# kurtosis/mat_mul

Hardware: NVIDIA B200
Metric: env_steps_per_sec (higher is better)
Workload: dtype int8

## Files before the change

### mat_mul_b200/csrc/tg_common.cuh

```cuda
#pragma once
#include <cuda_runtime.h>
#include <stdint.h>

#include <type_traits>

#include "../../include/tensorgame.h"

namespace tg {

template <int S>
struct Geo {
    static constexpr int S2 = S * S;
    static constexpr int S3 = S2 * S;
    static constexpr int RP = (S2 + 3) & ~3;
    static constexpr int WR = RP / 4;
    static constexpr int GP = (S * RP + 15) & ~15;
    static constexpr int TP = (3 * S + 15) & ~15;
    static constexpr bool STRADDLE = (S % 4) != 0;
};

__host__ __device__ constexpr bool supported_S(int S) { return S == 4 || S == 9 || S == 16 || S == 25; }
__host__ __device__ constexpr bool basis_supported_S(int S) { return S == 4 || S == 9 || S == 16; }

extern int g_last_cuda_error;

#ifdef TG_TUNING
}
#include <cstdlib>
namespace tg {
inline int tuning_env(const char *name, int dflt) {
    const char *e = getenv(name);
    return e ? atoi(e) : dflt;
}
#endif

inline int cuda_fail(cudaError_t e) {
    g_last_cuda_error = (int)e;
    return TG_E_CUDA;
}
#define TG_CUDA(call)                                  \
    do {                                               \
        cudaError_t _e = (call);                       \
        if (_e != cudaSuccess) return tg::cuda_fail(_e); \
    } while (0)

int sm_count();

template <class F>
int with_S(int S, F &&f) {
    switch (S) {
    case 4: return f(std::integral_constant<int, 4>{});
    case 9: return f(std::integral_constant<int, 9>{});
    case 16: return f(std::integral_constant<int, 16>{});
    case 25: return f(std::integral_constant<int, 25>{});
    }
    return TG_E_ARG;
}

constexpr int LAUNCH = 1;

inline bool misaligned(const void *p, uintptr_t align) { return ((uintptr_t)p & (align - 1)) != 0; }

inline int check_step(int S, long long B, int shift, const void *in, const void *tape, const void *out, const void *flags,
                      const void *nnz) {
    if (!supported_S(S) || B < 0 || shift < 1 || shift > 4) return TG_E_ARG;
    if (B == 0) return TG_OK;
    if (!in || !tape || !out || !flags || !nnz) return TG_E_ARG;
    if (misaligned(in, 16) || misaligned(out, 16) || misaligned(tape, 16)) return TG_E_ARG;
    return LAUNCH;
}

inline int check_expand(int S, long long B, int k, int shift, const void *parents, const void *tape, const void *children,
                        const void *flags, const void *nnz) {
    if (k < 1) return TG_E_ARG;
    return check_step(S, B, shift, parents, tape, children, flags, nnz);
}

inline int check_rollout(int S, long long B, int K, int shift, const void *in, const void *tape, long long stride, const void *out,
                         const void *flags, const void *nnz, const void *steps, bool freeze) {
    if (!supported_S(S) || B < 0 || K < 0 || shift < 1 || shift > 4) return TG_E_ARG;
    if (B == 0) return TG_OK;
    if (!in || !out || !flags || !nnz || (freeze && !steps) || (K > 0 && !tape)) return TG_E_ARG;
    if (misaligned(in, 16) || misaligned(out, 16) || misaligned(tape, 16) || (stride & 15)) return TG_E_ARG;
    return LAUNCH;
}

inline int check_pair(int S, long long B, const void *src, uintptr_t src_align, const void *dst, uintptr_t dst_align) {
    if (!supported_S(S) || B < 0) return TG_E_ARG;
    if (B == 0) return TG_OK;
    if (!src || !dst) return TG_E_ARG;
    if (misaligned(src, src_align) || misaligned(dst, dst_align)) return TG_E_ARG;
    return LAUNCH;
}

inline int check_basis_gf2(int S, long long N, const void *in, const void *mats, const void *out) {
    if (!supported_S(S) || N < 0) return TG_E_ARG;
    if (N == 0) return TG_OK;
    if (!in || !mats || !out) return TG_E_ARG;
    if (misaligned(in, 16) || misaligned(out, 16) || misaligned(mats, 4)) return TG_E_ARG;
    return LAUNCH;
}

inline int check_basis_factors_gf2(int S, long long N, int R, int shift_in, int shift_out, const void *tape_in, long long in_stride,
                                   const void *mats, const void *tape_out, long long out_stride) {
    if (!supported_S(S) || N < 0 || R < 1 || shift_in < 1 || shift_in > 4 || shift_out < 1 || shift_out > 4) return TG_E_ARG;
    if (N == 0) return TG_OK;
    if (!tape_in || !mats || !tape_out) return TG_E_ARG;
    if (misaligned(tape_in, 16) || misaligned(tape_out, 16) || (in_stride & 15) || (out_stride & 15) || misaligned(mats, 4)) return TG_E_ARG;
    return LAUNCH;
}

inline int check_sample_gf2(int S, long long N, double p_nonzero, const void *mats) {
    if (!supported_S(S) || N < 0 || !(p_nonzero >= 0.0 && p_nonzero <= 1.0)) return TG_E_ARG;
    if (N == 0) return TG_OK;
    if (!mats) return TG_E_ARG;
    if (misaligned(mats, 4)) return TG_E_ARG;
    return LAUNCH;
}

inline int check_demo_sample_gf2(int S, long long N, int R, int dim_t, int replay_shift, long long nb, const void *tape_dm,
                                 const void *targets, const void *idx, const void *states, const void *scalars, const void *actions,
                                 const void *rewards) {
    if (!supported_S(S) || N < 0 || R < 1 || dim_t < 1 || nb < 0) return TG_E_ARG;
    if (nb == 0) return TG_OK;
    if (!tape_dm || !targets || !idx || !states || !scalars || !actions || !rewards) return TG_E_ARG;
    if (misaligned(tape_dm, 16) || misaligned(targets, 16)) return TG_E_ARG;
    if (replay_shift < 0 || replay_shift > 8) return TG_E_ARG;
    return LAUNCH;
}

constexpr uint8_t BASIS_REDO = 0x80;
int launch_basis_mma16(const int8_t *slab_in, const int8_t *mats, long long mat_stride, void *slab_out, int out16, uint8_t *flags,
                       long long N, cudaStream_t st);
int launch_basis_mma9(const int8_t *slab_in, const int8_t *mats, long long mat_stride, void *slab_out, int out16, uint8_t *flags,
                      long long N, cudaStream_t st);

int launch_rollout_rows(const int8_t *slab_in, const uint8_t *tape, long long stride, int K, int8_t *slab_out, uint8_t *flags,
                        int32_t *nnz, int32_t *steps, long long B, int S, int shift, int freeze, cudaStream_t st);
bool demo_acc16_mma_applies(int R);
int launch_demo_acc16_mma(const uint8_t *tape, long long tape_step_stride, long long N, int R, int shift, int8_t *slab,
                          uint8_t *flags, int or_flags, cudaStream_t st);

__device__ __forceinline__ void philox_block(uint32_t c0, uint32_t c1, uint32_t c2, uint32_t c3, uint32_t k0, uint32_t k1,
                                             uint32_t out[4]) {
#pragma unroll
    for (int r = 0; r < 10; r++) {
        const uint32_t hi0 = __umulhi(0xD2511F53u, c0), lo0 = 0xD2511F53u * c0;
        const uint32_t hi1 = __umulhi(0xCD9E8D57u, c2), lo1 = 0xCD9E8D57u * c2;
        c0 = hi1 ^ c1 ^ k0, c1 = lo1, c2 = hi0 ^ c3 ^ k1, c3 = lo0;
        k0 += 0x9E3779B9u, k1 += 0xBB67AE85u;
    }
    out[0] = c0, out[1] = c1, out[2] = c2, out[3] = c3;
}

__device__ __forceinline__ unsigned long long splitmix64(unsigned long long z) {
    z += 0x9E3779B97F4A7C15ull;
    z = (z ^ (z >> 30)) * 0xBF58476D1CE4E5B9ull;
    z = (z ^ (z >> 27)) * 0x94D049BB133111EBull;
    return z ^ (z >> 31);
}
__device__ __forceinline__ unsigned long long key_const(unsigned base, int i) { return splitmix64((unsigned long long)(base + i)) | 1ull; }

__device__ __forceinline__ uint32_t smem_u32(const void *p) { return (uint32_t)__cvta_generic_to_shared(p); }

__device__ __forceinline__ void mbar_init(uint64_t *bar, uint32_t count) {
    asm volatile("mbarrier.init.shared::cta.b64 [%0], %1;" ::"r"(smem_u32(bar)), "r"(count));
}
__device__ __forceinline__ void mbar_fence_init() { asm volatile("fence.mbarrier_init.release.cluster;" ::: "memory"); }
__device__ __forceinline__ void mbar_expect_tx(uint64_t *bar, uint32_t bytes) {
    asm volatile("mbarrier.arrive.expect_tx.shared::cta.b64 _, [%0], %1;" ::"r"(smem_u32(bar)), "r"(bytes) : "memory");
}
__device__ __forceinline__ void mbar_wait(uint64_t *bar, uint32_t parity) {
    asm volatile(
        "{\n"
        ".reg .pred p;\n"
        "WAIT_%=:\n"
        "mbarrier.try_wait.parity.shared::cta.b64 p, [%0], %1;\n"
        "@p bra DONE_%=;\n"
        "bra WAIT_%=;\n"
        "DONE_%=:\n"
        "}\n" ::"r"(smem_u32(bar)),
        "r"(parity)
        : "memory");
}
__device__ __forceinline__ void bulk_g2s(void *dst_smem, const void *src_gmem, uint32_t bytes, uint64_t *bar) {
    asm volatile("cp.async.bulk.shared::cluster.global.mbarrier::complete_tx::bytes [%0], [%1], %2, [%3];" ::"r"(
                     smem_u32(dst_smem)),
                 "l"(src_gmem), "r"(bytes), "r"(smem_u32(bar))
                 : "memory");
}
__device__ __forceinline__ void bulk_s2g(void *dst_gmem, const void *src_smem, uint32_t bytes) {
    asm volatile("cp.async.bulk.global.shared::cta.bulk_group [%0], [%1], %2;" ::"l"(dst_gmem), "r"(smem_u32(src_smem)),
                 "r"(bytes)
                 : "memory");
}
__device__ __forceinline__ void bulk_commit() { asm volatile("cp.async.bulk.commit_group;" ::: "memory"); }
template <int N>
__device__ __forceinline__ void bulk_wait_read() {
    asm volatile("cp.async.bulk.wait_group.read %0;" ::"n"(N) : "memory");
}
template <int N>
__device__ __forceinline__ void bulk_wait() {
    asm volatile("cp.async.bulk.wait_group %0;" ::"n"(N) : "memory");
}
__device__ __forceinline__ void fence_proxy_async() { asm volatile("fence.proxy.async.shared::cta;" ::: "memory"); }

constexpr uint32_t H4 = 0x80808080u;
constexpr uint32_t ONES4 = 0x01010101u;

__device__ __forceinline__ uint32_t nonzero_mask(uint32_t x) { return (((x & 0x7F7F7F7Fu) + 0x7F7F7F7Fu) | x) & H4; }

__device__ __forceinline__ uint32_t byte_sum(uint32_t x) { return __dp4a(x, ONES4, 0u); }

__device__ __forceinline__ void st_f32x4(float *p, float a, float b, float c, float d) {
    asm volatile("st.global.v4.f32 [%0], {%1, %2, %3, %4};" ::"l"(__cvta_generic_to_global(p)), "f"(a), "f"(b), "f"(c), "f"(d) : "memory");
}
__device__ __forceinline__ void st_f32x2(float *p, float a, float b) {
    asm volatile("st.global.v2.f32 [%0], {%1, %2};" ::"l"(__cvta_generic_to_global(p)), "f"(a), "f"(b) : "memory");
}
__device__ __forceinline__ void st_f32(float *p, float a) {
    asm volatile("st.global.f32 [%0], %1;" ::"l"(__cvta_generic_to_global(p)), "f"(a) : "memory");
}
__device__ __forceinline__ void ld_f32x4(const float *p, float f[4]) {
    asm volatile("ld.global.nc.v4.f32 {%0, %1, %2, %3}, [%4];" : "=f"(f[0]), "=f"(f[1]), "=f"(f[2]), "=f"(f[3]) : "l"(__cvta_generic_to_global(p)));
}
__device__ __forceinline__ void ld_f32x2(const float *p, float &a, float &b) {
    asm volatile("ld.global.nc.v2.f32 {%0, %1}, [%2];" : "=f"(a), "=f"(b) : "l"(__cvta_generic_to_global(p)));
}
__device__ __forceinline__ float ld_f32(const float *p) {
    float a;
    asm volatile("ld.global.nc.f32 %0, [%1];" : "=f"(a) : "l"(__cvta_generic_to_global(p)));
    return a;
}

template <int S>
__device__ __forceinline__ void store_run(float *p, int nv, float a, float b, float c, float d) {
    const uint32_t lo = (uint32_t)reinterpret_cast<uintptr_t>(p);
    if constexpr (Geo<S>::S2 % 4 == 0) {
        if ((lo & 15u) == 0) {
            st_f32x4(p, a, b, c, d);
            return;
        }
    }
    if (nv == 4) {
        if ((lo & 7u) == 0) {
            st_f32x2(p, a, b);
            st_f32x2(p + 2, c, d);
        } else {
            st_f32(p, a);
            st_f32x2(p + 1, b, c);
            st_f32(p + 3, d);
        }
    } else {
        if (nv > 0) st_f32(p, a);
        if (nv > 1) st_f32(p + 1, b);
        if (nv > 2) st_f32(p + 2, c);
    }
}

template <int S>
__device__ __forceinline__ void load_run(const float *p, int nv, float f[4]) {
    const uint32_t lo = (uint32_t)reinterpret_cast<uintptr_t>(p);
    f[0] = f[1] = f[2] = f[3] = 0.f;
    if constexpr (Geo<S>::S2 % 4 == 0) {
        if ((lo & 15u) == 0) {
            ld_f32x4(p, f);
            return;
        }
    }
    if (nv == 4) {
        if ((lo & 7u) == 0) {
            ld_f32x2(p, f[0], f[1]);
            ld_f32x2(p + 2, f[2], f[3]);
        } else {
            f[0] = ld_f32(p);
            ld_f32x2(p + 1, f[1], f[2]);
            f[3] = ld_f32(p + 3);
        }
    } else {
        if (nv > 0) f[0] = ld_f32(p);
        if (nv > 1) f[1] = ld_f32(p + 1);
        if (nv > 2) f[2] = ld_f32(p + 2);
    }
}

}
```

### mat_mul_b200/csrc/tg_expand.cu

```cuda
#include "tg_step.cuh"

namespace tg {

template <int B>
__device__ __forceinline__ int sext_byte_e(uint32_t w) {
    constexpr uint32_t sel = (uint32_t)B | ((uint32_t)(B | 8) << 4) | ((uint32_t)(B | 8) << 8) | ((uint32_t)(B | 8) << 12);
    uint32_t d;
    asm("prmt.b32 %0, %1, %2, %3;" : "=r"(d) : "r"(w), "r"(0u), "r"(sel));
    return (int)d;
}
__device__ __forceinline__ unsigned long long quad_sum64(unsigned long long x) {
    x += __shfl_xor_sync(0xFFFFFFFFu, x, 1);
    x += __shfl_xor_sync(0xFFFFFFFFu, x, 2);
    return x;
}

template <bool KEYS>
__global__ void __launch_bounds__(128)
    expand4_rows_kernel(const int8_t *__restrict__ parents, const uint8_t *__restrict__ tape, int k, int8_t *__restrict__ children,
                        uint8_t *__restrict__ flags, int32_t *__restrict__ nnz, unsigned long long *__restrict__ keys, long long B,
                        int shift) {
    constexpr int S = 4;
    const long long gt = (long long)blockIdx.x * blockDim.x + threadIdx.x;
    const long long b = min(gt >> 2, B - 1);
    const bool real = (gt >> 2) < B;
    const int i = (int)(gt & 3);
    uint32_t row[4];
    {
        const uint4 t = __ldg(reinterpret_cast<const uint4 *>(parents + b * 64) + i);
        row[0] = t.x ^ H4, row[1] = t.y ^ H4, row[2] = t.z ^ H4, row[3] = t.w ^ H4;
    }
    unsigned long long pkey = 0;
    const unsigned long long Ai = i == 0 ? key_const(0x1000, 0) : i == 1 ? key_const(0x1000, 1) : i == 2 ? key_const(0x1000, 2) : key_const(0x1000, 3);
    if constexpr (KEYS) {
        unsigned long long ti = 0;
#pragma unroll
        for (int j = 0; j < S; j++) {
            const uint32_t w = row[j] ^ H4;
            unsigned long long sij = 0;
#pragma unroll
            for (int kk = 0; kk < S; kk++) sij += (unsigned long long)(long long)(int8_t)(w >> (8 * kk)) * key_const(0x3000, kk);
            ti += sij * key_const(0x2000, j);
        }
        pkey = quad_sum64(ti * Ai);
    }
    const uint32_t sh4 = (uint32_t)shift * ONES4, tokmax = (uint32_t)(0x7F - 2 * shift) * ONES4;
    const uint4 *rec = reinterpret_cast<const uint4 *>(tape + b * k * 16);
    uint4 *dst = reinterpret_cast<uint4 *>(children + b * k * 64) + i;
    const int ush = 8 * i;
    unsigned long long kc[S] = {0, 0, 0, 0};
    if constexpr (KEYS) {
#pragma unroll
        for (int x = 0; x < S; x++) kc[x] = key_const(0x1000u * (unsigned)(i + 1), x);
    }
    uint4 q = __ldg(rec);
    for (int c = 0; c < k; c++) {
        const uint4 cur = q;
        if (c + 1 < k) q = __ldg(rec + c + 1);
        const uint32_t over = ((((cur.x & 0x7F7F7F7Fu) + tokmax) | cur.x) | (((cur.y & 0x7F7F7F7Fu) + tokmax) | cur.y) |
                               (((cur.z & 0x7F7F7F7Fu) + tokmax) | cur.z)) & H4;
        const uint32_t cu = ((cur.x | H4) - sh4) ^ H4, cv = ((cur.y | H4) - sh4) ^ H4, cw = ((cur.z | H4) - sh4) ^ H4;
        const int wi = (int)(cur.z - sh4);
        const int ui = (int)(int8_t)(cu >> ush);
        const int v[4] = {sext_byte_e<0>(cv), sext_byte_e<1>(cv), sext_byte_e<2>(cv), sext_byte_e<3>(cv)};
        uint32_t part = 0, rng = 0;
        uint32_t t[4];
#pragma unroll
        for (int j = 0; j < 4; j++) {
            const uint32_t x = (row[j] - (uint32_t)(ui * v[j] * wi)) ^ H4;
            t[j] = x;
            part += (uint32_t)__popc(nonzero_mask(x));
            rng |= x ^ (x << 1);
        }
        if (real) dst[4 * c] = make_uint4(t[0], t[1], t[2], t[3]);
        part |= (rng & H4) != 0 ? 1u << 16 : 0u;
        part += __shfl_xor_sync(0xFFFFFFFFu, part, 1);
        part += __shfl_xor_sync(0xFFFFFFFFu, part, 2);
        unsigned long long fkey = 0;
        if constexpr (KEYS) {
            const uint32_t cm = i == 0 ? cu : (i == 1 ? cv : cw);
            unsigned long long f = 0;
#pragma unroll
            for (int x = 0; x < S; x++) f += (unsigned long long)(long long)(int8_t)(cm >> (8 * x)) * kc[x];
            const unsigned long long f1 = __shfl_sync(0xFFFFFFFFu, f, (threadIdx.x & 28) | 1);
            const unsigned long long f2 = __shfl_sync(0xFFFFFFFFu, f, (threadIdx.x & 28) | 2);
            fkey = f * f1 * f2;
        }
        if (real && i == 0) {
            const uint32_t cntv = part & 0xFFFFu;
            const bool changed = cu != 0 && cv != 0 && cw != 0;
            const long long child = b * k + c;
            flags[child] = (uint8_t)((cntv == 0 ? TG_FLAG_TERMINAL : 0u) | (changed ? 0u : TG_FLAG_NULL) |
                                     (((part >> 16) != 0 || over != 0) ? TG_FLAG_RANGE : 0u));
            nnz[child] = (int32_t)cntv;
            if constexpr (KEYS) keys[child] = pkey - fkey;
        }
    }
}

}

extern "C" int tg_expand_children(const int8_t *parents, const uint8_t *tape, int k, int8_t *children, uint8_t *flags,
                                  int32_t *nnz, uint64_t *keys, int64_t B, int S, int shift, void *stream) {
    if (const int rc = tg::check_expand(S, B, k, shift, parents, tape, children, flags, nnz); rc != tg::LAUNCH) return rc;
    cudaStream_t st = (cudaStream_t)stream;
    switch (S) {
    case 4: {
#ifdef TG_TUNING
        if (tg::tuning_env("TG_EXPAND_COLUMNS", 0))
            return tg::launch_expand<4, 256, tg::W8>(parents, tape, k, children, flags, nnz, (unsigned long long *)keys, B, shift, st);
#endif
        const long long grid = (B * 4 + 127) / 128;
        if (grid > 0x7FFFFFFFLL) return TG_E_ARG;
        if (keys) tg::expand4_rows_kernel<true><<<(int)grid, 128, 0, st>>>(parents, tape, k, children, flags, nnz, (unsigned long long *)keys, B, shift);
        else tg::expand4_rows_kernel<false><<<(int)grid, 128, 0, st>>>(parents, tape, k, children, flags, nnz, nullptr, B, shift);
        TG_CUDA(cudaGetLastError());
        return TG_OK;
    }
    case 9: return tg::launch_expand<9, 128, tg::W8>(parents, tape, k, children, flags, nnz, (unsigned long long *)keys, B, shift, st);
    case 16: return tg::launch_expand<16, 128, tg::W8>(parents, tape, k, children, flags, nnz, (unsigned long long *)keys, B, shift, st);
    case 25: return tg::launch_expand<25, 160, tg::W8>(parents, tape, k, children, flags, nnz, (unsigned long long *)keys, B, shift, st);
    }
    return TG_E_ARG;
}
```

### mat_mul_b200/csrc/tg_step.cu

```cuda
#include "tg_step.cuh"

namespace tg {

int g_last_cuda_error = 0;

int sm_count() {
    static int cached[64] = {0};
    int dev = 0;
    if (cudaGetDevice(&dev) != cudaSuccess || dev < 0 || dev >= 64) return 148;
    if (!cached[dev]) {
        int n = 0;
        if (cudaDeviceGetAttribute(&n, cudaDevAttrMultiProcessorCount, dev) != cudaSuccess || n <= 0) n = 148;
        cached[dev] = n;
    }
    return cached[dev];
}

#ifdef TG_TUNING
static int g_step_ctas_per_sm = 0;
static int g_step_variant = 0;
#endif

static int step_ctas_per_sm(int n) {
#ifdef TG_TUNING
    if (g_step_ctas_per_sm > 0) return g_step_ctas_per_sm;
#endif
    return n;
}

}

extern "C" {

int tg_version(void) { return TG_VERSION; }
int tg_last_cuda_error(void) { return tg::g_last_cuda_error; }

const char *tg_error_string(int code) {
    switch (code) {
    case TG_OK: return "ok";
    case TG_E_ARG: return "bad argument";
    case TG_E_CUDA: return "CUDA runtime error (see tg_last_cuda_error)";
    case TG_E_RANGE: return "value does not fit the device format";
    default: return "unknown error";
    }
}

int tg_layout(int S, int *row_pitch, int *game_pitch, int *token_pitch) {
    if (!tg::supported_S(S)) return TG_E_ARG;
    const int rp = (S * S + 3) & ~3;
    if (row_pitch) *row_pitch = rp;
    if (game_pitch) *game_pitch = (S * rp + 15) & ~15;
    if (token_pitch) *token_pitch = (3 * S + 15) & ~15;
    return TG_OK;
}

#ifdef TG_TUNING
int tg_tune_step_ctas_per_sm(int n) {
    tg::g_step_ctas_per_sm = n;
    return TG_OK;
}
int tg_tune_step_variant(int v) {
    tg::g_step_variant = v;
    return TG_OK;
}
#endif

int tg_step(const int8_t *slab_in, const uint8_t *tape, int8_t *slab_out, uint8_t *flags, int32_t *nnz, int64_t B, int S,
            int shift, void *stream) {
    if (const int rc = tg::check_step(S, B, shift, slab_in, tape, slab_out, flags, nnz); rc != tg::LAUNCH) return rc;
    cudaStream_t st = (cudaStream_t)stream;
#ifdef TG_TUNING
    switch (S * 10 + tg::g_step_variant) {
    case 41: return tg::launch_step<4, 256, 2, 2, tg::W8>(slab_in, tape, slab_out, flags, nnz, B, shift, tg::step_ctas_per_sm(32), st);
    case 42: return tg::launch_step<4, 256, 4, 3, tg::W8>(slab_in, tape, slab_out, flags, nnz, B, shift, tg::step_ctas_per_sm(32), st);
    case 43: return tg::launch_step<4, 256, 8, 2, tg::W8>(slab_in, tape, slab_out, flags, nnz, B, shift, tg::step_ctas_per_sm(32), st);
    case 91: return tg::launch_step<9, 256, 1, 3, tg::W8>(slab_in, tape, slab_out, flags, nnz, B, shift, tg::step_ctas_per_sm(5), st);
    case 92: return tg::launch_step<9, 256, 1, 4, tg::W8>(slab_in, tape, slab_out, flags, nnz, B, shift, tg::step_ctas_per_sm(5), st);
    case 93: return tg::launch_step<9, 256, 4, 2, tg::W8>(slab_in, tape, slab_out, flags, nnz, B, shift, tg::step_ctas_per_sm(32), st);
    case 94: return tg::launch_step<9, 512, 1, 3, tg::W8>(slab_in, tape, slab_out, flags, nnz, B, shift, tg::step_ctas_per_sm(3), st);
    case 95: return tg::launch_step<9, 128, 2, 3, tg::W8>(slab_in, tape, slab_out, flags, nnz, B, shift, tg::step_ctas_per_sm(7), st);
    case 96: return tg::launch_step<9, 128, 4, 3, tg::W8>(slab_in, tape, slab_out, flags, nnz, B, shift, tg::step_ctas_per_sm(5), st);
    case 97: return tg::launch_step<9, 256, 2, 3, tg::W8>(slab_in, tape, slab_out, flags, nnz, B, shift, tg::step_ctas_per_sm(32), st);
    case 161: return tg::launch_step<16, 256, 1, 3, tg::W8>(slab_in, tape, slab_out, flags, nnz, B, shift, tg::step_ctas_per_sm(32), st);
    case 162: return tg::launch_step<16, 256, 2, 2, tg::W8>(slab_in, tape, slab_out, flags, nnz, B, shift, tg::step_ctas_per_sm(32), st);
    case 163: return tg::launch_step<16, 512, 1, 2, tg::W8>(slab_in, tape, slab_out, flags, nnz, B, shift, tg::step_ctas_per_sm(32), st);
    default: break;
    }
#endif
    switch (S) {
    case 4: return tg::launch_step<4, 256, 4, 2, tg::W8>(slab_in, tape, slab_out, flags, nnz, B, shift, tg::step_ctas_per_sm(32), st);
    case 9: return tg::launch_step<9, 256, 2, 2, tg::W8>(slab_in, tape, slab_out, flags, nnz, B, shift, tg::step_ctas_per_sm(32), st);
    case 16: return tg::launch_step<16, 256, 1, 2, tg::W8>(slab_in, tape, slab_out, flags, nnz, B, shift, tg::step_ctas_per_sm(32), st);
    case 25: return tg::launch_step<25, 160, 1, 2, tg::W8>(slab_in, tape, slab_out, flags, nnz, B, shift, tg::step_ctas_per_sm(32), st);
    }
    return TG_E_ARG;
}

}
```

### mat_mul_b200/csrc/tg_step.cuh

```cuda
#pragma once
#include "tg_common.cuh"

namespace tg {

struct W8 {
    using T = int8_t;
    static constexpr int EB = 1;
    static constexpr uint32_t H = H4;
    static constexpr int NB = 16, CB = 8;
    static constexpr bool UNROLL_PASSES = true;

    template <int S>
    struct Lane {
        int c;
        uint32_t hv;
        uint32_t maskA;
        uint32_t maskB;
        int off_vA, off_vB;
        int off_w[4];
        int tokw;

        __device__ __forceinline__ void init(int c_) {
            using G = Geo<S>;
            c = c_;
            tokw = c_ % (G::TP / 4);
            const int jk0 = 4 * c;
            const int jA = jk0 / S;
            hv = 0, maskA = 0, maskB = 0;
#pragma unroll
            for (int b = 0; b < 4; b++) {
                const int jk = jk0 + b;
                const bool valid = jk < G::S2;
                const int j = valid ? jk / S : jA;
                const int k = valid ? jk % S : 0;
                off_w[b] = 2 * S + k;
                if (valid) {
                    hv |= 0x80u << (8 * b);
                    if (j == jA)
                        maskA |= 0xFFu << (8 * b);
                    else
                        maskB |= 0xFFu << (8 * b);
                }
            }
            off_vA = S + jA;
            off_vB = S + (jA + 1 < S ? jA + 1 : jA);
        }
    };

    template <int S>
    static __device__ __forceinline__ int32_t pack_vw(const uint8_t *tok, const Lane<S> &L, int shift) {
        using G = Geo<S>;
        const int vA = (int)tok[L.off_vA] - shift;
        if constexpr (!G::STRADDLE) {
            const uint32_t wt = *reinterpret_cast<const uint32_t *>(tok + L.off_w[0]);
            return vA * (int32_t)(wt - (uint32_t)shift * ONES4);
        } else {
            const int vB = (int)tok[L.off_vB] - shift;
            const uint32_t wt = (uint32_t)tok[L.off_w[0]] | ((uint32_t)tok[L.off_w[1]] << 8) |
                                ((uint32_t)tok[L.off_w[2]] << 16) | ((uint32_t)tok[L.off_w[3]] << 24);
            const uint32_t sh = (uint32_t)shift * ONES4, mv = L.maskA | L.maskB;
            const int32_t ws = (int32_t)((wt & mv) - (sh & mv));
            const int32_t wsB = (int32_t)((wt & L.maskB) - (sh & L.maskB));
            return vA * ws + (vB - vA) * wsB;
        }
    }

    static __device__ __forceinline__ uint32_t lane_sum(uint32_t cnt) { return byte_sum(cnt); }

    template <int S>
    struct ColumnKey {
        unsigned long long kb[4];

        __device__ __forceinline__ void init(int c) {
#pragma unroll
            for (int q = 0; q < 4; q++) {
                const int jk = 4 * c + q;
                kb[q] = jk < Geo<S>::S2 ? key_const(0x2000, jk / S) * key_const(0x3000, jk % S) : 0ull;
            }
        }
        __device__ __forceinline__ unsigned long long operator()(const uint32_t (&row)[S]) const {
            unsigned long long a0 = 0;
#pragma unroll
            for (int i = 0; i < S; i++) a0 -= 128ull * key_const(0x1000, i);
            unsigned long long acc[4] = {a0, a0, a0, a0};
#pragma unroll
            for (int i = 0; i < S; i++) {
#pragma unroll
                for (int q = 0; q < 4; q++) acc[q] += (unsigned long long)((row[i] >> (8 * q)) & 0xFFu) * key_const(0x1000, i);
            }
            return acc[0] * kb[0] + acc[1] * kb[1] + acc[2] * kb[2] + acc[3] * kb[3];
        }
    };
};

struct W16 {
    using T = int16_t;
    static constexpr int EB = 2;
    static constexpr uint32_t H = 0x80008000u;
    static constexpr int NB = 14, CB = 9;
    static constexpr bool UNROLL_PASSES = false;

    template <int S>
    struct Lane {
        int c;
        uint32_t hv;
        int off_v[2], off_w[2];
        int m1;
        int tokw;

        __device__ __forceinline__ void init(int c_) {
            c = c_;
            tokw = c_ % (Geo<S>::TP / 4);
            hv = 0;
#pragma unroll
            for (int b = 0; b < 2; b++) {
                const int jk = 2 * c + b;
                const bool valid = jk < Geo<S>::S2;
                off_v[b] = S + (valid ? jk / S : 0);
                off_w[b] = 2 * S + (valid ? jk % S : 0);
                if (valid) hv |= 0x8000u << (16 * b);
            }
            m1 = (hv >> 31) & 1;
        }
    };

    template <int S>
    static __device__ __forceinline__ uint32_t pack_vw(const uint8_t *tok, const Lane<S> &L, int shift) {
        const int d0 = ((int)tok[L.off_v[0]] - shift) * ((int)tok[L.off_w[0]] - shift);
        const int d1 = ((int)tok[L.off_v[1]] - shift) * ((int)tok[L.off_w[1]] - shift);
        return L.hv ? (uint32_t)d0 + ((uint32_t)(d1 * L.m1) << 16) : 0u;
    }

    static __device__ __forceinline__ uint32_t lane_sum(uint32_t cnt) { return (cnt & 0xFFFFu) + (cnt >> 16); }

    template <int S>
    struct ColumnKey {
        int c;

        __device__ __forceinline__ void init(int c_) { c = c_; }
        __device__ __forceinline__ unsigned long long operator()(const uint32_t (&row)[S]) const {
            unsigned long long a0 = 0;
#pragma unroll
            for (int i = 0; i < S; i++) a0 -= 32768ull * key_const(0x1000, i);
            unsigned long long acc[2] = {a0, a0};
#pragma unroll
            for (int i = 0; i < S; i++) {
                acc[0] += (unsigned long long)(row[i] & 0xFFFFu) * key_const(0x1000, i);
                acc[1] += (unsigned long long)(row[i] >> 16) * key_const(0x1000, i);
            }
            unsigned long long h = 0;
#pragma unroll
            for (int q = 0; q < 2; q++) {
                const int jk = 2 * c + q;
                if (jk < Geo<S>::S2) h += acc[q] * (key_const(0x2000, jk / S) * key_const(0x3000, jk % S));
            }
            return h;
        }
    };
};

template <int S>
using Lane = W8::Lane<S>;

template <int S, class F>
struct GeoW : Geo<S> {
    static constexpr int WR = Geo<S>::RP * F::EB / 4;
    static constexpr int GB = Geo<S>::GP * F::EB;
};

template <class F>
constexpr bool partial_fits = Geo<25>::S3 < (1 << F::NB) && GeoW<25, F>::WR < (1 << F::CB);
static_assert(partial_fits<W8> && partial_fits<W16>, "partial result word fields");

template <class F = W8>
__device__ __forceinline__ uint32_t make_partial(uint32_t nnz, bool changed, bool range) {
    return nnz | (changed ? 1u << F::NB : 0u) | (range ? 1u << (F::NB + F::CB) : 0u);
}
template <class F = W8>
__device__ __forceinline__ uint32_t partial_nnz(uint32_t sum) { return sum & ((1u << F::NB) - 1u); }
template <class F = W8>
__device__ __forceinline__ uint32_t partial_flags(uint32_t sum) {
    return (partial_nnz<F>(sum) == 0 ? TG_FLAG_TERMINAL : 0u) | (((sum >> F::NB) & ((1u << F::CB) - 1u)) == 0 ? TG_FLAG_NULL : 0u) |
           ((sum >> (F::NB + F::CB)) != 0 ? TG_FLAG_RANGE : 0u);
}

template <class F>
__device__ __forceinline__ uint32_t nonzero_lanes(uint32_t t, uint32_t hv) {
    return ((((t & ~F::H) + ~F::H) | t) & hv) >> (8 * F::EB - 1);
}

template <int S, class F = W8>
__device__ __forceinline__ bool tokens_out_of_range(const uint8_t *tok, const typename F::template Lane<S> &L, int shift) {
    static_assert(GeoW<S, F>::WR >= Geo<S>::TP / 4, "not enough threads per game to cover the token record");
    const uint32_t x = reinterpret_cast<const uint32_t *>(tok)[L.tokw];
    return ((((x & 0x7F7F7F7Fu) + (uint32_t)(0x7F - 2 * shift) * ONES4) | x) & H4) != 0;
}

template <int S>
constexpr int UW = 4 * ((S + 15) / 16);
template <int S>
__device__ __forceinline__ void load_u(const uint8_t *tok, uint32_t (&uw)[UW<S>]) {
    static_assert(UW<S> * 4 <= Geo<S>::TP, "u words inside the token record");
#pragma unroll
    for (int q = 0; q < UW<S> / 4; q++) {
        const uint4 ut = reinterpret_cast<const uint4 *>(tok)[q];
        uw[4 * q] = ut.x, uw[4 * q + 1] = ut.y, uw[4 * q + 2] = ut.z, uw[4 * q + 3] = ut.w;
    }
}

__device__ __forceinline__ int coef_u(const uint32_t *uw, int i, int shift) {
    return (int)__dp4a(uw[i >> 2], 1u << (8 * (i & 3)), (uint32_t)(-shift));
}

template <int S, int SIGN, class F = W8>
__device__ __forceinline__ uint32_t rank1_update(uint8_t *game, const uint8_t *tok, const typename F::template Lane<S> &L, int shift) {
    using G = GeoW<S, F>;
    const auto vw = F::template pack_vw<S>(tok, L, shift);
    uint32_t uw[UW<S>];
    load_u<S>(tok, uw);
    uint32_t cnt = 0, rng = 0;
    int uany = 0;
    uint32_t *col = reinterpret_cast<uint32_t *>(game) + L.c;
    const uint32_t svw = (uint32_t)(SIGN < 0 ? -vw : vw);
#pragma unroll
    for (int i = 0; i < S; i++) {
        const int negu = coef_u(uw, i, shift);
        uint32_t t = col[i * G::WR] ^ F::H;
        t += (uint32_t)negu * svw;
        t ^= F::H;
        col[i * G::WR] = t;
        cnt += nonzero_lanes<F>(t, L.hv);
        rng |= t ^ (t << 1);
        uany |= negu;
    }
    return make_partial<F>(F::lane_sum(cnt), vw != 0 && uany != 0, (rng & L.hv) != 0 || tokens_out_of_range<S, F>(tok, L, shift));
}

template <int S>
__device__ __forceinline__ uint32_t scan_game(const uint8_t *game, const Lane<S> &L) {
    using G = Geo<S>;
    uint32_t cnt = 0, rng = 0;
    const uint32_t *col = reinterpret_cast<const uint32_t *>(game) + L.c;
#pragma unroll
    for (int i = 0; i < S; i++) {
        const uint32_t t = col[i * G::WR];
        cnt += ((((t & 0x7F7F7F7Fu) + 0x7F7F7F7Fu) | t) & L.hv) >> 7;
        rng |= t ^ (t << 1);
    }
    return make_partial(byte_sum(cnt), true, (rng & L.hv) != 0);
}

template <int S, int NT, int NPASS, int NSTAGE, class F>
struct StepCfg {
    using G = GeoW<S, F>;
    static constexpr int GPASS = NT / G::WR;
    static constexpr int TG = GPASS * NPASS;
    static constexpr int ACTIVE = GPASS * G::WR;
    static constexpr int SLAB_BYTES = TG * G::GB;
    static constexpr int TOK_BYTES = TG * G::TP;
    static constexpr int STAGE_BYTES = SLAB_BYTES + TOK_BYTES;
    static constexpr int PW = (G::WR % 32 == 0) ? G::WR / 32 : ((32 % G::WR == 0) ? 1 : G::WR);
    static constexpr int PART_WORDS = TG * PW;
    static constexpr int SMEM_BYTES = NSTAGE * STAGE_BYTES + 2 * PART_WORDS * 4 + 2 * NSTAGE * 8;
    static constexpr int THREADS = NT + 32;
    static_assert(SMEM_BYTES <= 227 * 1024, "shared memory of one CTA");
};

template <int S, int NT, int NPASS, int NSTAGE, class F>
__global__ void __launch_bounds__(NT + 32)
    step_kernel(const typename F::T *__restrict__ slab_in, const uint8_t *__restrict__ tape, typename F::T *__restrict__ slab_out,
                uint8_t *__restrict__ flags, int32_t *__restrict__ nnz, long long B, int shift) {
    using C = StepCfg<S, NT, NPASS, NSTAGE, F>;
    using G = GeoW<S, F>;
    extern __shared__ __align__(128) uint8_t smem[];
    uint32_t *part = reinterpret_cast<uint32_t *>(smem + NSTAGE * C::STAGE_BYTES);
    uint64_t *full = reinterpret_cast<uint64_t *>(part + 2 * C::PART_WORDS);
    uint64_t *done = full + NSTAGE;

    const int tid = threadIdx.x;
    const long long ntiles = (B + C::TG - 1) / C::TG;

    if (tid == 0) {
        for (int s = 0; s < NSTAGE; s++) {
            mbar_init(&full[s], 1);
            mbar_init(&done[s], 1);
        }
        mbar_fence_init();
    }
    __syncthreads();

    if (tid >= NT) {
        if (tid != NT) return;
        auto load = [&](long long tile, int s) {
            const long long g0 = tile * C::TG;
            const int ng = (int)min((long long)C::TG, B - g0);
            uint8_t *st = smem + s * C::STAGE_BYTES;
            mbar_expect_tx(&full[s], (uint32_t)(ng * (G::GB + G::TP)));
            bulk_g2s(st, slab_in + g0 * G::GP, (uint32_t)(ng * G::GB), &full[s]);
            bulk_g2s(st + C::SLAB_BYTES, tape + g0 * G::TP, (uint32_t)(ng * G::TP), &full[s]);
        };
        long long tile = blockIdx.x;
        for (int s = 0; s < NSTAGE && tile + (long long)s * gridDim.x < ntiles; s++) load(tile + (long long)s * gridDim.x, s);
        for (int it = 0; tile < ntiles; tile += gridDim.x, it++) {
            const int s = it % NSTAGE;
            const uint32_t parity = (uint32_t)(it / NSTAGE) & 1u;
            mbar_wait(&done[s], parity);
            const long long g0 = tile * C::TG;
            const int ng = (int)min((long long)C::TG, B - g0);
            bulk_s2g(slab_out + g0 * G::GP, smem + s * C::STAGE_BYTES, (uint32_t)(ng * G::GB));
            bulk_commit();
            const long long next = tile + (long long)NSTAGE * gridDim.x;
            if (next < ntiles) {
                bulk_wait_read<0>();
                load(next, s);
            }
        }
        bulk_wait<0>();
        return;
    }

    typename F::template Lane<S> L;
    const bool active = tid < C::ACTIVE;
    const int gl = tid / G::WR;
    L.init(active ? tid % G::WR : 0);

    int it = 0;
    for (long long tile = blockIdx.x; tile < ntiles; tile += gridDim.x, it++) {
        const int s = it % NSTAGE;
        const uint32_t parity = (uint32_t)(it / NSTAGE) & 1u;
        const long long g0 = tile * C::TG;
        const int ng = (int)min((long long)C::TG, B - g0);
        uint8_t *slab = smem + s * C::STAGE_BYTES;
        const uint8_t *toks = slab + C::SLAB_BYTES;
        uint32_t *pp = part + (it & 1) * C::PART_WORDS;

        mbar_wait(&full[s], parity);
        if constexpr (F::UNROLL_PASSES) {
#pragma unroll
            for (int p = 0; p < NPASS; p++) {
                const int g = p * C::GPASS + gl;
                uint32_t pr = 0;
                if (active && g < ng) pr = rank1_update<S, -1, F>(slab + g * G::GB, toks + g * G::TP, L, shift);
                if constexpr (G::WR % 32 == 0) {
                    pr = __reduce_add_sync(0xFFFFFFFFu, pr);
                    if ((tid & 31) == 0 && g < ng) pp[g * C::PW + (tid % G::WR) / 32] = pr;
                } else if constexpr (32 % G::WR == 0) {
#pragma unroll
                    for (int o = 1; o < G::WR; o <<= 1) pr += __shfl_xor_sync(0xFFFFFFFFu, pr, o);
                    if (L.c == 0 && g < ng) pp[g] = pr;
                } else {
                    if (active && g < ng) pp[g * C::PW + L.c] = pr;
                }
            }
        } else {
#pragma unroll 1
            for (int p = 0; p < NPASS; p++) {
                const int g = p * C::GPASS + gl;
                uint32_t pr = 0;
                if (active && g < ng) pr = rank1_update<S, -1, F>(slab + g * G::GB, toks + g * G::TP, L, shift);
                if constexpr (G::WR % 32 == 0) {
                    pr = __reduce_add_sync(0xFFFFFFFFu, pr);
                    if ((tid & 31) == 0 && g < ng) pp[g * C::PW + (tid % G::WR) / 32] = pr;
                } else if constexpr (32 % G::WR == 0) {
#pragma unroll
                    for (int o = 1; o < G::WR; o <<= 1) pr += __shfl_xor_sync(0xFFFFFFFFu, pr, o);
                    if (L.c == 0 && g < ng) pp[g] = pr;
                } else {
                    if (active && g < ng) pp[g * C::PW + L.c] = pr;
                }
            }
        }
        fence_proxy_async();
        asm volatile("bar.sync 1, %0;" ::"n"(NT) : "memory");
        if (tid == 0) asm volatile("mbarrier.arrive.shared::cta.b64 _, [%0];" ::"r"(smem_u32(&done[s])) : "memory");
        for (int g = tid; g < ng; g += NT) {
            uint32_t sum = 0;
#pragma unroll
            for (int w = 0; w < C::PW; w++) sum += pp[g * C::PW + w];
            flags[g0 + g] = (uint8_t)partial_flags<F>(sum);
            nnz[g0 + g] = (int32_t)partial_nnz<F>(sum);
        }
    }
}

template <int S, int NT, int NPASS, int NSTAGE, class F>
int launch_step(const typename F::T *slab_in, const uint8_t *tape, typename F::T *slab_out, uint8_t *flags, int32_t *nnz,
                long long B, int shift, int ctas_per_sm, cudaStream_t stream) {
    using C = StepCfg<S, NT, NPASS, NSTAGE, F>;
    auto kern = step_kernel<S, NT, NPASS, NSTAGE, F>;
    TG_CUDA(cudaFuncSetAttribute(kern, cudaFuncAttributeMaxDynamicSharedMemorySize, C::SMEM_BYTES));
    const long long ntiles = (B + C::TG - 1) / C::TG;
    const long long cap = (long long)sm_count() * ctas_per_sm;
    const int grid = (int)(ntiles < cap ? ntiles : cap);
    kern<<<grid, C::THREADS, C::SMEM_BYTES, stream>>>(slab_in, tape, slab_out, flags, nnz, B, shift);
    TG_CUDA(cudaGetLastError());
    return TG_OK;
}

template <int S, int NT, class F>
struct ExpCfg {
    using G = GeoW<S, F>;
    static constexpr int TG = NT / G::WR;
    static constexpr int ACTIVE = TG * G::WR;
    static constexpr int STAGE_BYTES = TG * G::GB;
    static __host__ __device__ constexpr int tok_bytes(int k) { return (TG * k * G::TP + 15) & ~15; }
    static constexpr int NSTAGE = 3;
    static __host__ __device__ constexpr int smem_bytes(int k) {
        return tok_bytes(k) + NSTAGE * STAGE_BYTES + ((NSTAGE * TG * 4 + 7) & ~7) + TG * 8 + 16 + NT * 8;
    }
};

template <int S, int NT, bool KEYS, class F>
__global__ void __launch_bounds__(NT)
    expand_kernel(const typename F::T *__restrict__ parents, const uint8_t *__restrict__ tape, int k,
                  typename F::T *__restrict__ children, uint8_t *__restrict__ flags, int32_t *__restrict__ nnz,
                  unsigned long long *__restrict__ keys, long long B, int shift) {
    using C = ExpCfg<S, NT, F>;
    using G = GeoW<S, F>;
    extern __shared__ __align__(128) uint8_t smem[];
    uint8_t *s_tok = smem;
    constexpr int NSTAGE = C::NSTAGE;
    uint8_t *s_out = smem + C::tok_bytes(k);
    uint32_t *s_part = reinterpret_cast<uint32_t *>(s_out + NSTAGE * C::STAGE_BYTES);
    unsigned long long *s_pkey = reinterpret_cast<unsigned long long *>(reinterpret_cast<uint8_t *>(s_part) + ((NSTAGE * C::TG * 4 + 7) & ~7));
    uint64_t *s_bar = reinterpret_cast<uint64_t *>(s_pkey + C::TG);
    unsigned long long *s_ph = reinterpret_cast<unsigned long long *>(s_bar + 2);
    uint8_t *out = reinterpret_cast<uint8_t *>(children);

    const int tid = threadIdx.x;
    const long long g0 = (long long)blockIdx.x * C::TG;
    const int ng = (int)min((long long)C::TG, B - g0);
    const int g = tid / G::WR;
    const bool active = tid < C::ACTIVE && g < ng;
    typename F::template Lane<S> L;
    L.init(tid < C::ACTIVE ? tid % G::WR : 0);

    if (tid == 0) {
        mbar_init(s_bar, 1);
        mbar_fence_init();
    }
    for (int w = tid; w < NSTAGE * C::STAGE_BYTES / 4; w += NT) reinterpret_cast<uint32_t *>(s_out)[w] = 0;
    for (int i = tid; i < NSTAGE * C::TG; i += NT) s_part[i] = 0;
    typename F::template ColumnKey<S> ck;
    if constexpr (KEYS) ck.init(L.c);
    __syncthreads();
    if (tid == 0) {
        mbar_expect_tx(s_bar, (uint32_t)(ng * k * G::TP));
        bulk_g2s(s_tok, tape + g0 * k * G::TP, (uint32_t)(ng * k * G::TP), s_bar);
    }
    uint32_t row[S];
    if (active) {
        const uint32_t *src = reinterpret_cast<const uint32_t *>(parents + (g0 + g) * G::GP) + L.c;
#pragma unroll
        for (int i = 0; i < S; i++) row[i] = src[i * G::WR] ^ F::H;
    } else {
#pragma unroll
        for (int i = 0; i < S; i++) row[i] = F::H;
    }
    if constexpr (KEYS) s_ph[tid] = ck(row);
    mbar_wait(s_bar, 0);
    if constexpr (KEYS) {
        __syncthreads();
        if (tid < ng) {
            unsigned long long h = 0;
            for (int c = 0; c < G::WR; c++) h += s_ph[tid * G::WR + c];
            s_pkey[tid] = h;
        }
        __syncthreads();
        for (int x = tid; x < ng * k; x += NT) {
            const uint8_t *tok = s_tok + (size_t)x * G::TP;
            unsigned long long f[3];
#pragma unroll
            for (int m = 0; m < 3; m++) {
                unsigned long long a = 0;
#pragma unroll
                for (int i = 0; i < S; i++) a += (unsigned long long)(long long)((int)tok[m * S + i] - shift) * key_const(0x1000 * (m + 1), i);
                f[m] = a;
            }
            keys[g0 * k + x] = s_pkey[x / k] - f[0] * f[1] * f[2];
        }
    }

    for (int c = 0, st = 0; c < k; c++, st = st + 1 == NSTAGE ? 0 : st + 1) {
        uint8_t *stage = s_out + st * C::STAGE_BYTES;
        if (active) {
            const uint8_t *tok = s_tok + ((size_t)g * k + c) * G::TP;
            const auto vw = F::template pack_vw<S>(tok, L, shift);
            uint32_t uw[UW<S>];
            load_u<S>(tok, uw);
            const uint32_t nvw = (uint32_t)(-vw);
            uint32_t cnt = 0, rng = 0;
            int uany = 0;
            uint32_t *col = reinterpret_cast<uint32_t *>(stage + (size_t)g * G::GB) + L.c;
#pragma unroll
            for (int i = 0; i < S; i++) {
                const int negu = coef_u(uw, i, shift);
                const uint32_t t = (row[i] + (uint32_t)negu * nvw) ^ F::H;
                col[i * G::WR] = t;
                cnt += nonzero_lanes<F>(t, L.hv);
                rng |= t ^ (t << 1);
                uany |= negu;
            }
            atomicAdd(&s_part[st * C::TG + g], make_partial<F>(F::lane_sum(cnt), vw != 0 && uany != 0,
                                                               (rng & L.hv) != 0 || tokens_out_of_range<S, F>(tok, L, shift)));
        }
        fence_proxy_async();
        __syncthreads();
        if (tid < ng) {
            const long long child = (g0 + tid) * k + c;
            bulk_s2g(out + child * G::GB, stage + (size_t)tid * G::GB, (uint32_t)G::GB);
            bulk_commit();
            const uint32_t sum = s_part[st * C::TG + tid];
            flags[child] = (uint8_t)partial_flags<F>(sum);
            nnz[child] = (int32_t)partial_nnz<F>(sum);
            s_part[st * C::TG + tid] = 0;
            bulk_wait_read<1>();
        }
    }
    if (tid < ng) bulk_wait<0>();
}

template <int S, int NT, class F>
int launch_expand(const typename F::T *parents, const uint8_t *tape, int k, typename F::T *children, uint8_t *flags, int32_t *nnz,
                  unsigned long long *keys, long long B, int shift, cudaStream_t st) {
    using C = ExpCfg<S, NT, F>;
    if (k > (200 * 1024 - C::smem_bytes(0)) / (C::TG * Geo<S>::TP)) return TG_E_ARG;
    const int smem = C::smem_bytes(k);
    const long long grid = (B + C::TG - 1) / C::TG;
    if (grid > 0x7FFFFFFFLL) return TG_E_ARG;
    if (keys) {
        auto kern = expand_kernel<S, NT, true, F>;
        TG_CUDA(cudaFuncSetAttribute(kern, cudaFuncAttributeMaxDynamicSharedMemorySize, smem));
        kern<<<(int)grid, NT, smem, st>>>(parents, tape, k, children, flags, nnz, keys, B, shift);
    } else {
        auto kern = expand_kernel<S, NT, false, F>;
        TG_CUDA(cudaFuncSetAttribute(kern, cudaFuncAttributeMaxDynamicSharedMemorySize, smem));
        kern<<<(int)grid, NT, smem, st>>>(parents, tape, k, children, flags, nnz, keys, B, shift);
    }
    TG_CUDA(cudaGetLastError());
    return TG_OK;
}
}
```

Measured before the change: 4.173 billion.

## Add row-per-thread S=4 step kernel and alternate traversal direction for L2 reuse

Replaces the TMA-pipelined column step kernel for S=4 with a simple register-only kernel where each quad of threads handles one game. Each thread loads its row and the tape record directly, and the kernel batches G games per warp. It also adds a host-side heuristic that reverses tile traversal order when consecutive steps ping-pong buffers, so the most recently written data, likely still in L2, is read first. The row update math moves into a shared helper that uses byte_perm and folded multiplies, and the expand kernel reuses it. The direction heuristic relies on host-side pointer tracking via static atomics.

Result: no change. 4.146 billion (median of 6 runs) (-0.6%).

```diff
diff --git a/mat_mul_b200/csrc/tg_common.cuh b/mat_mul_b200/csrc/tg_common.cuh
--- a/mat_mul_b200/csrc/tg_common.cuh
+++ b/mat_mul_b200/csrc/tg_common.cuh
@@ -45,6 +45,7 @@
     } while (0)
 
 int sm_count();
+int step_direction(const void *slab_in, const void *slab_out);
 
 template <class F>
 int with_S(int S, F &&f) {
diff --git a/mat_mul_b200/csrc/tg_expand.cu b/mat_mul_b200/csrc/tg_expand.cu
--- a/mat_mul_b200/csrc/tg_expand.cu
+++ b/mat_mul_b200/csrc/tg_expand.cu
@@ -2,13 +2,6 @@
 
 namespace tg {
 
-template <int B>
-__device__ __forceinline__ int sext_byte_e(uint32_t w) {
-    constexpr uint32_t sel = (uint32_t)B | ((uint32_t)(B | 8) << 4) | ((uint32_t)(B | 8) << 8) | ((uint32_t)(B | 8) << 12);
-    uint32_t d;
-    asm("prmt.b32 %0, %1, %2, %3;" : "=r"(d) : "r"(w), "r"(0u), "r"(sel));
-    return (int)d;
-}
 __device__ __forceinline__ unsigned long long quad_sum64(unsigned long long x) {
     x += __shfl_xor_sync(0xFFFFFFFFu, x, 1);
     x += __shfl_xor_sync(0xFFFFFFFFu, x, 2);
@@ -44,10 +37,8 @@
         }
         pkey = quad_sum64(ti * Ai);
     }
-    const uint32_t sh4 = (uint32_t)shift * ONES4, tokmax = (uint32_t)(0x7F - 2 * shift) * ONES4;
     const uint4 *rec = reinterpret_cast<const uint4 *>(tape + b * k * 16);
     uint4 *dst = reinterpret_cast<uint4 *>(children + b * k * 64) + i;
-    const int ush = 8 * i;
     unsigned long long kc[S] = {0, 0, 0, 0};
     if constexpr (KEYS) {
 #pragma unroll
@@ -57,28 +48,14 @@
     for (int c = 0; c < k; c++) {
         const uint4 cur = q;
         if (c + 1 < k) q = __ldg(rec + c + 1);
-        const uint32_t over = ((((cur.x & 0x7F7F7F7Fu) + tokmax) | cur.x) | (((cur.y & 0x7F7F7F7Fu) + tokmax) | cur.y) |
-                               (((cur.z & 0x7F7F7F7Fu) + tokmax) | cur.z)) & H4;
-        const uint32_t cu = ((cur.x | H4) - sh4) ^ H4, cv = ((cur.y | H4) - sh4) ^ H4, cw = ((cur.z | H4) - sh4) ^ H4;
-        const int wi = (int)(cur.z - sh4);
-        const int ui = (int)(int8_t)(cu >> ush);
-        const int v[4] = {sext_byte_e<0>(cv), sext_byte_e<1>(cv), sext_byte_e<2>(cv), sext_byte_e<3>(cv)};
-        uint32_t part = 0, rng = 0;
         uint32_t t[4];
-#pragma unroll
-        for (int j = 0; j < 4; j++) {
-            const uint32_t x = (row[j] - (uint32_t)(ui * v[j] * wi)) ^ H4;
-            t[j] = x;
-            part += (uint32_t)__popc(nonzero_mask(x));
-            rng |= x ^ (x << 1);
-        }
+        bool null;
+        const uint32_t part = quad_sum(step_row4(row, cur, i, shift, t, null));
         if (real) dst[4 * c] = make_uint4(t[0], t[1], t[2], t[3]);
-        part |= (rng & H4) != 0 ? 1u << 16 : 0u;
-        part += __shfl_xor_sync(0xFFFFFFFFu, part, 1);
-        part += __shfl_xor_sync(0xFFFFFFFFu, part, 2);
         unsigned long long fkey = 0;
         if constexpr (KEYS) {
-            const uint32_t cm = i == 0 ? cu : (i == 1 ? cv : cw);
+            const uint32_t sh4 = (uint32_t)shift * ONES4;
+            const uint32_t cm = ((((i == 0 ? cur.x : (i == 1 ? cur.y : cur.z)) | H4) - sh4) ^ H4);
             unsigned long long f = 0;
 #pragma unroll
             for (int x = 0; x < S; x++) f += (unsigned long long)(long long)(int8_t)(cm >> (8 * x)) * kc[x];
@@ -87,12 +64,9 @@
             fkey = f * f1 * f2;
         }
         if (real && i == 0) {
-            const uint32_t cntv = part & 0xFFFFu;
-            const bool changed = cu != 0 && cv != 0 && cw != 0;
             const long long child = b * k + c;
-            flags[child] = (uint8_t)((cntv == 0 ? TG_FLAG_TERMINAL : 0u) | (changed ? 0u : TG_FLAG_NULL) |
-                                     (((part >> 16) != 0 || over != 0) ? TG_FLAG_RANGE : 0u));
-            nnz[child] = (int32_t)cntv;
+            flags[child] = quad_flags(part, null);
+            nnz[child] = (int32_t)(part & 0xFFFFu);
             if constexpr (KEYS) keys[child] = pkey - fkey;
         }
     }
diff --git a/mat_mul_b200/csrc/tg_step.cu b/mat_mul_b200/csrc/tg_step.cu
--- a/mat_mul_b200/csrc/tg_step.cu
+++ b/mat_mul_b200/csrc/tg_step.cu
@@ -1,4 +1,6 @@
 #include "tg_step.cuh"
+
+#include <atomic>
 
 namespace tg {
 
@@ -16,6 +18,20 @@
     return cached[dev];
 }
 
+int step_direction(const void *slab_in, const void *slab_out) {
+    static std::atomic<uintptr_t> last_out[64];
+    static std::atomic<int> last_rev[64];
+    int dev = 0;
+    if (cudaGetDevice(&dev) != cudaSuccess || dev < 0 || dev >= 64) return 0;
+#ifdef TG_TUNING
+    if (tuning_env("TG_STEP_FORWARD", 0)) return 0;
+#endif
+    const int rev = (uintptr_t)slab_in == last_out[dev].load(std::memory_order_relaxed) && !last_rev[dev].load(std::memory_order_relaxed);
+    last_out[dev].store((uintptr_t)slab_out, std::memory_order_relaxed);
+    last_rev[dev].store(rev, std::memory_order_relaxed);
+    return rev;
+}
+
 #ifdef TG_TUNING
 static int g_step_ctas_per_sm = 0;
 static int g_step_variant = 0;
@@ -27,6 +43,67 @@
 #endif
     return n;
 }
+
+template <int G, int NT>
+__global__ void __launch_bounds__(NT)
+    step4_rows_kernel(const int8_t *slab_in, const uint8_t *tape, int8_t *slab_out, uint8_t *flags, int32_t *nnz, long long B, int shift,
+                      int rev) {
+    const int lane = threadIdx.x & 31, i = lane & 3;
+    const long long nwarps = (long long)gridDim.x * (NT / 32), nchunks = (B + 8 * G - 1) / (8 * G);
+    for (long long w = (long long)blockIdx.x * (NT / 32) + threadIdx.x / 32; w < nchunks; w += nwarps) {
+        const long long b0 = (rev ? nchunks - 1 - w : w) * (8 * G) + (lane >> 2);
+        uint4 in[G], rec[G];
+#pragma unroll
+        for (int g = 0; g < G; g++) {
+            const long long b = b0 + 8 * g;
+            in[g] = b < B ? reinterpret_cast<const uint4 *>(slab_in + b * 64)[i] : make_uint4(0u, 0u, 0u, 0u);
+            rec[g] = b < B ? __ldg(reinterpret_cast<const uint4 *>(tape) + b) : make_uint4(0u, 0u, 0u, 0u);
+        }
+#pragma unroll
+        for (int g = 0; g < G; g++) {
+            const long long b = b0 + 8 * g;
+            const uint32_t row[4] = {in[g].x ^ H4, in[g].y ^ H4, in[g].z ^ H4, in[g].w ^ H4};
+            uint32_t t[4];
+            bool null;
+            const uint32_t part = quad_sum(step_row4(row, rec[g], i, shift, t, null));
+            if (b < B) {
+                reinterpret_cast<uint4 *>(slab_out + b * 64)[i] = make_uint4(t[0], t[1], t[2], t[3]);
+                if (i == 0) {
+                    flags[b] = quad_flags(part, null);
+                    nnz[b] = (int32_t)(part & 0xFFFFu);
+                }
+            }
+        }
+    }
+}
+
+template <int G, int NT>
+int launch_step4(const int8_t *slab_in, const uint8_t *tape, int8_t *slab_out, uint8_t *flags, int32_t *nnz, long long B, int shift,
+                 int ctas_per_sm, cudaStream_t stream) {
+    constexpr int GAMES = NT / 4 * G;
+    const long long need = (B + GAMES - 1) / GAMES;
+    const long long cap = (long long)sm_count() * ctas_per_sm;
+    const int rev = step_direction(slab_in, slab_out);
+    step4_rows_kernel<G, NT><<<(int)(need < cap ? need : cap), NT, 0, stream>>>(slab_in, tape, slab_out, flags, nnz, B, shift, rev);
+    TG_CUDA(cudaGetLastError());
+    return TG_OK;
+}
+
+#ifdef TG_TUNING
+static int step4_tuned(const int8_t *in, const uint8_t *tape, int8_t *out, uint8_t *flags, int32_t *nnz, long long B, int shift,
+                       cudaStream_t st) {
+    const int G = tuning_env("TG_STEP4_G", 0), NT = tuning_env("TG_STEP4_NT", 0);
+    switch (G * 1000 + NT) {
+    case 1128: return launch_step4<1, 128>(in, tape, out, flags, nnz, B, shift, step_ctas_per_sm(32), st);
+    case 1256: return launch_step4<1, 256>(in, tape, out, flags, nnz, B, shift, step_ctas_per_sm(32), st);
+    case 2128: return launch_step4<2, 128>(in, tape, out, flags, nnz, B, shift, step_ctas_per_sm(32), st);
+    case 2256: return launch_step4<2, 256>(in, tape, out, flags, nnz, B, shift, step_ctas_per_sm(32), st);
+    case 4128: return launch_step4<4, 128>(in, tape, out, flags, nnz, B, shift, step_ctas_per_sm(32), st);
+    case 4256: return launch_step4<4, 256>(in, tape, out, flags, nnz, B, shift, step_ctas_per_sm(32), st);
+    }
+    return -1;
+}
+#endif
 
 }
 
@@ -88,7 +165,14 @@
     }
 #endif
     switch (S) {
-    case 4: return tg::launch_step<4, 256, 4, 2, tg::W8>(slab_in, tape, slab_out, flags, nnz, B, shift, tg::step_ctas_per_sm(32), st);
+    case 4: {
+#ifdef TG_TUNING
+        if (tg::tuning_env("TG_STEP_COLUMNS", 0))
+            return tg::launch_step<4, 256, 4, 2, tg::W8>(slab_in, tape, slab_out, flags, nnz, B, shift, tg::step_ctas_per_sm(32), st);
+        if (const int rc = tg::step4_tuned(slab_in, tape, slab_out, flags, nnz, B, shift, st); rc != -1) return rc;
+#endif
+        return tg::launch_step4<2, 256>(slab_in, tape, slab_out, flags, nnz, B, shift, tg::step_ctas_per_sm(32), st);
+    }
     case 9: return tg::launch_step<9, 256, 2, 2, tg::W8>(slab_in, tape, slab_out, flags, nnz, B, shift, tg::step_ctas_per_sm(32), st);
     case 16: return tg::launch_step<16, 256, 1, 2, tg::W8>(slab_in, tape, slab_out, flags, nnz, B, shift, tg::step_ctas_per_sm(32), st);
     case 25: return tg::launch_step<25, 160, 1, 2, tg::W8>(slab_in, tape, slab_out, flags, nnz, B, shift, tg::step_ctas_per_sm(32), st);
diff --git a/mat_mul_b200/csrc/tg_step.cuh b/mat_mul_b200/csrc/tg_step.cuh
--- a/mat_mul_b200/csrc/tg_step.cuh
+++ b/mat_mul_b200/csrc/tg_step.cuh
@@ -250,6 +250,37 @@
     return make_partial(byte_sum(cnt), true, (rng & L.hv) != 0);
 }
 
+__device__ __forceinline__ uint32_t step_row4(const uint32_t (&row)[4], const uint4 rec, int i, int shift, uint32_t (&t)[4], bool &null) {
+    const uint32_t sh4 = (uint32_t)shift * ONES4;
+    const uint32_t W = rec.z - sh4;
+    const uint32_t nsW = (uint32_t)(-shift) * W;
+    const uint32_t negu = (uint32_t)shift - __byte_perm(rec.x, 0u, 0x4440u | (uint32_t)i);
+    const uint32_t ri = i == 0 ? rec.x : i == 1 ? rec.y : i == 2 ? rec.z : rec.w;
+    const uint32_t over = (((ri & 0x7F7F7F7Fu) + (uint32_t)(0x7F - 2 * shift) * ONES4) | ri) & H4;
+    uint32_t cnt = 0, rng = 0, vwany = 0;
+#pragma unroll
+    for (int j = 0; j < 4; j++) {
+        const uint32_t vW = __byte_perm(rec.y, 0u, 0x4440u | (uint32_t)j) * W + nsW;
+        const uint32_t x = (row[j] + negu * vW) ^ H4;
+        t[j] = x;
+        cnt += (uint32_t)__popc(nonzero_mask(x));
+        rng |= x ^ (x << 1);
+        vwany |= vW;
+    }
+    null = rec.x == sh4 || vwany == 0;
+    return cnt | ((rng & H4) != 0 || over != 0 ? 1u << 16 : 0u);
+}
+
+__device__ __forceinline__ uint32_t quad_sum(uint32_t x) {
+    x += __shfl_xor_sync(0xFFFFFFFFu, x, 1);
+    x += __shfl_xor_sync(0xFFFFFFFFu, x, 2);
+    return x;
+}
+
+__device__ __forceinline__ uint8_t quad_flags(uint32_t part, bool null) {
+    return (uint8_t)(((part & 0xFFFFu) == 0 ? TG_FLAG_TERMINAL : 0u) | (null ? TG_FLAG_NULL : 0u) | ((part >> 16) != 0 ? TG_FLAG_RANGE : 0u));
+}
+
 template <int S, int NT, int NPASS, int NSTAGE, class F>
 struct StepCfg {
     using G = GeoW<S, F>;
@@ -269,7 +300,7 @@
 template <int S, int NT, int NPASS, int NSTAGE, class F>
 __global__ void __launch_bounds__(NT + 32)
     step_kernel(const typename F::T *__restrict__ slab_in, const uint8_t *__restrict__ tape, typename F::T *__restrict__ slab_out,
-                uint8_t *__restrict__ flags, int32_t *__restrict__ nnz, long long B, int shift) {
+                uint8_t *__restrict__ flags, int32_t *__restrict__ nnz, long long B, int shift, int rev) {
     using C = StepCfg<S, NT, NPASS, NSTAGE, F>;
     using G = GeoW<S, F>;
     extern __shared__ __align__(128) uint8_t smem[];
@@ -279,6 +310,7 @@
 
     const int tid = threadIdx.x;
     const long long ntiles = (B + C::TG - 1) / C::TG;
+    auto first_game = [&](long long tile) { return (rev ? ntiles - 1 - tile : tile) * C::TG; };
 
     if (tid == 0) {
         for (int s = 0; s < NSTAGE; s++) {
@@ -292,7 +324,7 @@
     if (tid >= NT) {
         if (tid != NT) return;
         auto load = [&](long long tile, int s) {
-            const long long g0 = tile * C::TG;
+            const long long g0 = first_game(tile);
             const int ng = (int)min((long long)C::TG, B - g0);
             uint8_t *st = smem + s * C::STAGE_BYTES;
             mbar_expect_tx(&full[s], (uint32_t)(ng * (G::GB + G::TP)));
@@ -305,7 +337,7 @@
             const int s = it % NSTAGE;
             const uint32_t parity = (uint32_t)(it / NSTAGE) & 1u;
             mbar_wait(&done[s], parity);
-            const long long g0 = tile * C::TG;
+            const long long g0 = first_game(tile);
             const int ng = (int)min((long long)C::TG, B - g0);
             bulk_s2g(slab_out + g0 * G::GP, smem + s * C::STAGE_BYTES, (uint32_t)(ng * G::GB));
             bulk_commit();
@@ -328,7 +360,7 @@
     for (long long tile = blockIdx.x; tile < ntiles; tile += gridDim.x, it++) {
         const int s = it % NSTAGE;
         const uint32_t parity = (uint32_t)(it / NSTAGE) & 1u;
-        const long long g0 = tile * C::TG;
+        const long long g0 = first_game(tile);
         const int ng = (int)min((long long)C::TG, B - g0);
         uint8_t *slab = smem + s * C::STAGE_BYTES;
         const uint8_t *toks = slab + C::SLAB_BYTES;
@@ -386,13 +418,14 @@
 template <int S, int NT, int NPASS, int NSTAGE, class F>
 int launch_step(const typename F::T *slab_in, const uint8_t *tape, typename F::T *slab_out, uint8_t *flags, int32_t *nnz,
                 long long B, int shift, int ctas_per_sm, cudaStream_t stream) {
+    const int rev = step_direction(slab_in, slab_out);
     using C = StepCfg<S, NT, NPASS, NSTAGE, F>;
     auto kern = step_kernel<S, NT, NPASS, NSTAGE, F>;
     TG_CUDA(cudaFuncSetAttribute(kern, cudaFuncAttributeMaxDynamicSharedMemorySize, C::SMEM_BYTES));
     const long long ntiles = (B + C::TG - 1) / C::TG;
     const long long cap = (long long)sm_count() * ctas_per_sm;
     const int grid = (int)(ntiles < cap ? ntiles : cap);
-    kern<<<grid, C::THREADS, C::SMEM_BYTES, stream>>>(slab_in, tape, slab_out, flags, nnz, B, shift);
+    kern<<<grid, C::THREADS, C::SMEM_BYTES, stream>>>(slab_in, tape, slab_out, flags, nnz, B, shift, rev);
     TG_CUDA(cudaGetLastError());
     return TG_OK;
 }
```
